# chao-ji/ldm_tf2

Hardware: AMD Instinct MI355X
Metric: images/sec (256x256, 200 DDIM steps, CFG=5) (higher is better)
Workload: dtype bf16

## Files before the change

ldm_tf2_amd/csrc/attention.hip:

```cpp
#include "common.h"
#include <atomic>
#include <stdlib.h>

namespace {

struct AttnArgs {
  const char* q; const char* k; const char* vt; char* out;
  int64_t ldq, q_bs, ldk, k_bs, ldvt, vt_bs, ldo, o_bs;
  int heads, Tq, Tk;
  float scale;
};

__device__ __forceinline__ void mma32a(f32x16& acc, const u32x4& a, const u32x4& b, bf16_t) {
  acc = __builtin_amdgcn_mfma_f32_32x32x16_bf16(__builtin_bit_cast(bf16x8, a),
                                                __builtin_bit_cast(bf16x8, b), acc, 0, 0, 0);
}
__device__ __forceinline__ void mma32a(f32x16& acc, const u32x4& a, const u32x4& b, float) {
#pragma unroll
  for (int j = 0; j < 4; ++j)
    acc = __builtin_amdgcn_mfma_f32_32x32x2f32(__uint_as_float(a[j]), __uint_as_float(b[j]), acc,
                                               0, 0, 0);
}


template <typename T>
__device__ __forceinline__ u32x4 keep_first(u32x4 v, int nvalid) {
  constexpr int EPW = 4 / (int)sizeof(T);
#pragma unroll
  for (int w = 0; w < 4; ++w) {
    const int left = nvalid - w * EPW;
    if (left <= 0) v[w] = 0u;
    else if (EPW == 2 && left == 1) v[w] &= 0xffffu;
  }
  return v;
}

template <typename T> struct AttnTraits;
template <> struct AttnTraits<bf16_t> {
  static constexpr int NPC = 2;
  __device__ static __forceinline__ int kappa(int i) {
    return (i & ~12) | ((i & 4) << 1) | ((i & 8) >> 1);
  }
  __device__ static __forceinline__ u32x4 pchunk(const f32x16& s, int pc) {
    u32x4 c;
#pragma unroll
    for (int e = 0; e < 4; ++e) c[e] = pack_bf2(s[8 * pc + 2 * e], s[8 * pc + 2 * e + 1]);
    return c;
  }
};
template <> struct AttnTraits<float> {
  static constexpr int NPC = 4;
  __device__ static __forceinline__ int kappa(int i) { return i; }
  __device__ static __forceinline__ u32x4 pchunk(const f32x16& s, int pc) {
    u32x4 c;
#pragma unroll
    for (int e = 0; e < 4; ++e) c[e] = __float_as_uint(s[4 * pc + e]);
    return c;
  }
};

template <typename T, int SP, int KT, bool MS = false, int NWV = 4, int PF = 1>
__global__ __launch_bounds__(64 * NWV, (sizeof(T) == 2 ? (SP == 32 ? 3 : SP <= 64 ? 4 : 1) : 1)) void attn_kernel(AttnArgs p) {
  constexpr int NT = 64 * NWV;
  static_assert((NWV == 4 || NWV == 8) && (PF == 1 || PF == 2), "attention workgroup shape");
  using TR = AttnTraits<T>;
  constexpr int EPC = Elem<T>::kPerChunk;
  constexpr int NPC = TR::NPC;
  constexpr int NSUB = KT / 32;
  constexpr int DCH = SP / EPC;
  constexpr int VCH = KT / EPC;
  constexpr int NKG = SP * (int)sizeof(T) / 32;
  constexpr int ND = (SP + 31) / 32;
  constexpr int KRS = SP * (int)sizeof(T) + 16;
  constexpr int VRS = KT * (int)sizeof(T) + 16;
  constexpr int CK = (KT * DCH + NT - 1) / NT;
  constexpr int CV = (SP * VCH + NT - 1) / NT;
  static_assert(SP % 16 == 0 && KT % 32 == 0 && (SP * (int)sizeof(T)) % 32 == 0, "attention tile");

  __shared__ __attribute__((aligned(16))) char smem[KT * KRS + ND * 32 * VRS];
  char* sK = smem;
  char* sV = smem + KT * KRS;

  const int tid = threadIdx.x, lane = tid & 63, wave = tid >> 6;
  const int lr = lane & 31, lh = lane >> 5;
  const int head = blockIdx.y, b = blockIdx.z;
  const int q0 = blockIdx.x * (32 * NWV) + wave * 32;

  const T* Q = (const T*)p.q + (int64_t)b * p.q_bs + (int64_t)head * SP;
  const T* Kp = (const T*)p.k + (int64_t)b * p.k_bs + (int64_t)head * SP;
  const T* Vt = (const T*)p.vt + (int64_t)b * p.vt_bs + (int64_t)head * SP * p.ldvt;

  u32x4 qf[NKG];
  {
    const int qi = min(q0 + lr, p.Tq - 1);
    const T* qr = Q + (int64_t)qi * p.ldq;
#pragma unroll
    for (int g = 0; g < NKG; ++g) qf[g] = *(const u32x4*)(qr + (2 * g + lh) * EPC);
  }

  f32x16 o[ND];
#pragma unroll
  for (int d = 0; d < ND; ++d)
#pragma unroll
    for (int r = 0; r < 16; ++r) o[d][r] = 0.f;
  constexpr int RD = 40;
  static_assert(!MS || (sizeof(T) == 2 && SP == 48), "matrix-side softmax: bf16, 40-wide heads padded to 48");
  float m_run = MS ? 0.f : -INFINITY, l_run = 0.f;
  const float c2 = p.scale * 1.4426950408889634f;

  u32x4 rkA[CK], rvA[CV];
  [[maybe_unused]] u32x4 rkB[PF == 2 ? CK : 1], rvB[PF == 2 ? CV : 1];
  auto load_tile = [&](int kt0, u32x4 (&rk)[CK], u32x4 (&rv)[CV]) {
#pragma unroll
    for (int i = 0; i < CK; ++i) {
      const int id = tid + i * NT;
      const int key = id / DCH, dc = id - key * DCH;
      u32x4 v = {0u, 0u, 0u, 0u};
      if (id < KT * DCH && kt0 + key < p.Tk)
        v = *(const u32x4*)(Kp + (int64_t)(kt0 + key) * p.ldk + dc * EPC);
      rk[i] = v;
    }
#pragma unroll
    for (int i = 0; i < CV; ++i) {
      const int id = tid + i * NT;
      const int dim = id / VCH, kc = id - dim * VCH;
      u32x4 v = {0u, 0u, 0u, 0u};
      const int left = p.Tk - (kt0 + kc * EPC);
      if (id < SP * VCH && left > 0) {
        v = *(const u32x4*)(Vt + (int64_t)dim * p.ldvt + kt0 + kc * EPC);
        if (left < EPC) v = keep_first<T>(v, left);
      }
      rv[i] = v;
    }
  };
  auto store_tile = [&](const u32x4 (&rk)[CK], const u32x4 (&rv)[CV]) {
#pragma unroll
    for (int i = 0; i < CK; ++i) {
      const int id = tid + i * NT;
      const int key = id / DCH, dc = id - key * DCH;
      if (id < KT * DCH) *(u32x4*)(sK + key * KRS + dc * 16) = rk[i];
    }
#pragma unroll
    for (int i = 0; i < CV; ++i) {
      const int id = tid + i * NT;
      const int dim = id / VCH, kc = id - dim * VCH;
      if (id < SP * VCH) *(u32x4*)(sV + dim * VRS + kc * 16) = rv[i];
    }
  };

  const int krow = TR::kappa(lr);
  const int ntiles = (p.Tk + KT - 1) / KT;
  auto tile_body = [&](int t) {
    const int kt0 = t * KT;

    f32x16 s[NSUB];
#pragma unroll
    for (int j = 0; j < NSUB; ++j) {
#pragma unroll
      for (int r = 0; r < 16; ++r) s[j][r] = 0.f;
      const char* kr = sK + (j * 32 + krow) * KRS + lh * 16;
#pragma unroll
      for (int g = 0; g < NKG; ++g) {
        const u32x4 kf = *(const u32x4*)(kr + g * 32);
        mma32a(s[j], kf, qf[g], T());
      }
    }
    if (kt0 + KT > p.Tk) {
#pragma unroll
      for (int j = 0; j < NSUB; ++j)
#pragma unroll
        for (int r = 0; r < 16; ++r) {
          const int key = kt0 + j * 32 + TR::kappa((r & 3) + 8 * (r >> 2) + 4 * lh);
          if (key >= p.Tk) s[j][r] = -INFINITY;
        }
    }
    if constexpr (MS) {
      float mt = -INFINITY;
#pragma unroll
      for (int j = 0; j < NSUB; ++j)
#pragma unroll
        for (int r = 0; r < 16; r += 2) mt = fmaxf(fmaxf(mt, s[j][r]), s[j][r + 1]);
      mt = fmaxf(mt, __shfl_xor(mt, 32, 64));
      if (t == 0 || !__all(mt <= 8.0f)) {
        const float want = m_run + (t == 0 ? mt : fmaxf(mt, 0.f));
        const float m_new = bf2f(f2bf(want));
        const float delta = m_new - m_run;
        m_run = m_new;
        if (t > 0) {
          const float alpha = __builtin_amdgcn_exp2f(-delta);
#pragma unroll
          for (int d = 0; d < ND; ++d)
#pragma unroll
            for (int r = 0; r < 16; ++r) o[d][r] *= alpha;
        }
#pragma unroll
        for (int j = 0; j < NSUB; ++j)
#pragma unroll
          for (int r = 0; r < 16; ++r) s[j][r] -= delta;
        if (lh == (RD % 16) / 8) {
          uint32_t w = qf[RD / 16][(RD % 8) / 2];
          const uint32_t nb = (uint32_t)f2bf(-m_new);
          w = (RD % 2) ? ((w & 0x0000ffffu) | (nb << 16)) : ((w & 0xffff0000u) | nb);
          qf[RD / 16][(RD % 8) / 2] = w;
        }
      }
#pragma unroll
      for (int j = 0; j < NSUB; ++j)
#pragma unroll
        for (int r = 0; r < 16; ++r) s[j][r] = __builtin_amdgcn_exp2f(s[j][r]);
    } else {
    float mt = -INFINITY;
#pragma unroll
    for (int j = 0; j < NSUB; ++j)
#pragma unroll
      for (int r = 0; r < 16; ++r) mt = fmaxf(mt, s[j][r]);
    mt = fmaxf(mt, __shfl_xor(mt, 32, 64)) * c2;
    if (!__all(mt <= m_run + 8.0f)) {
      const float m_new = fmaxf(m_run, mt);
      const float alpha = __builtin_amdgcn_exp2f(m_run - m_new);
      m_run = m_new;
      l_run *= alpha;
#pragma unroll
      for (int d = 0; d < ND; ++d)
#pragma unroll
        for (int r = 0; r < 16; ++r) o[d][r] *= alpha;
    }
    float ls = 0.f;
#pragma unroll
    for (int j = 0; j < NSUB; ++j)
#pragma unroll
      for (int r = 0; r < 16; ++r) {
        const float e = __builtin_amdgcn_exp2f(__builtin_fmaf(s[j][r], c2, -m_run));
        s[j][r] = e;
        ls += e;
      }
    l_run += ls;
    }
#pragma unroll
    for (int j = 0; j < NSUB; ++j)
#pragma unroll
      for (int pc = 0; pc < NPC; ++pc) {
        const u32x4 pf = TR::pchunk(s[j], pc);
        const int coff = (j * 2 * NPC + 2 * pc + lh) * 16;
#pragma unroll
        for (int d = 0; d < ND; ++d) {
          const u32x4 vf = *(const u32x4*)(sV + (d * 32 + lr) * VRS + coff);
          mma32a(o[d], vf, pf, T());
        }
      }
  };

  load_tile(0, rkA, rvA);
  if constexpr (PF == 2) {
    if (ntiles > 1) load_tile(KT, rkB, rvB);
    for (int t = 0; t < ntiles; t += 2) {
      __syncthreads();
      store_tile(rkA, rvA);
      __syncthreads();
      if (t + 2 < ntiles) load_tile((t + 2) * KT, rkA, rvA);
      tile_body(t);
      if (t + 1 < ntiles) {
        __syncthreads();
        store_tile(rkB, rvB);
        __syncthreads();
        if (t + 3 < ntiles) load_tile((t + 3) * KT, rkB, rvB);
        tile_body(t + 1);
      }
    }
  } else {
    for (int t = 0; t < ntiles; ++t) {
      __syncthreads();
      store_tile(rkA, rvA);
      __syncthreads();
      if (t + 1 < ntiles) load_tile((t + 1) * KT, rkA, rvA);
      tile_body(t);
    }
  }

  float l_tot;
  if constexpr (MS) {
    constexpr int RR = RD % 32;
    static_assert((RR % 8) < 4, "row RD must live in the lh = 0 half");
    l_tot = __shfl(o[RD / 32][(RR % 4) + 4 * (RR / 8)], lane & 31, 64);
  } else {
    l_tot = l_run + __shfl_xor(l_run, 32, 64);
  }
  const float inv = 1.0f / l_tot;
  const int qi = q0 + lr;
  if (qi < p.Tq) {
    T* orow = (T*)p.out + (int64_t)b * p.o_bs + (int64_t)qi * p.ldo + (int64_t)head * SP;
#pragma unroll
    for (int d = 0; d < ND; ++d)
#pragma unroll
      for (int r4 = 0; r4 < 4; ++r4) {
        const int dim = d * 32 + 8 * r4 + 4 * lh;
        if (dim >= SP) continue;
        float v[4];
#pragma unroll
        for (int e = 0; e < 4; ++e) v[e] = o[d][r4 * 4 + e] * inv;
        if constexpr (MS) {
#pragma unroll
          for (int e = 0; e < 4; ++e) v[e] = (dim + e == RD) ? 0.f : v[e];
        }
        if constexpr (sizeof(T) == 2) {
          u32x2 pk; pk[0] = pack_bf2(v[0], v[1]); pk[1] = pack_bf2(v[2], v[3]);
          *(u32x2*)(orow + dim) = pk;
        } else {
          f32x4 pk = {v[0], v[1], v[2], v[3]};
          *(f32x4*)(orow + dim) = pk;
        }
      }
  }
}



template <typename T>
__global__ __launch_bounds__(256) void attn_wide_kernel(AttnArgs p) {
  using TR = AttnTraits<T>;
  constexpr int EPC = Elem<T>::kPerChunk;
  constexpr int NPC = TR::NPC;
  constexpr int SP = 512, SPW = 128, KT = 32;
  constexpr int ES = (int)sizeof(T);
  constexpr int DCH = SP / EPC;
  constexpr int VCH = KT / EPC;
  constexpr int NKGW = SPW * ES / 32;
  constexpr int NDW = SPW / 32;
  constexpr int KRS = SP * ES + 16;
  constexpr int VRS = KT * ES + 16;
  constexpr int CK = KT * DCH / 256;
  constexpr int CV = SP * VCH / 256;
  static_assert((KT * DCH) % 256 == 0 && (SP * VCH) % 256 == 0, "staging");
  extern __shared__ __attribute__((aligned(16))) char smem_w[];
  char* sK = smem_w;
  char* sV = sK + KT * KRS;
  float* sX = (float*)(sV + SP * VRS);

  const int tid = threadIdx.x, lane = tid & 63, wave = tid >> 6;
  const int lr = lane & 31, lh = lane >> 5;
  const int head = blockIdx.y, b = blockIdx.z;
  const int q0 = blockIdx.x * 32;
  const T* Q = (const T*)p.q + (int64_t)b * p.q_bs + (int64_t)head * SP;
  const T* Kp = (const T*)p.k + (int64_t)b * p.k_bs + (int64_t)head * SP;
  const T* Vt = (const T*)p.vt + (int64_t)b * p.vt_bs + (int64_t)head * SP * p.ldvt;

  u32x4 qf[NKGW];
  {
    const int qi = min(q0 + lr, p.Tq - 1);
    const T* qr = Q + (int64_t)qi * p.ldq + wave * SPW;
#pragma unroll
    for (int g = 0; g < NKGW; ++g) qf[g] = *(const u32x4*)(qr + (2 * g + lh) * EPC);
  }
  f32x16 o[NDW];
#pragma unroll
  for (int d = 0; d < NDW; ++d)
#pragma unroll
    for (int r = 0; r < 16; ++r) o[d][r] = 0.f;
  float m_run = -INFINITY, l_run = 0.f;
  const float c2 = p.scale * 1.4426950408889634f;
  const int krow = TR::kappa(lr);
  const int ntiles = (p.Tk + KT - 1) / KT;
  for (int t = 0; t < ntiles; ++t) {
    const int kt0 = t * KT;
    __syncthreads();
#pragma unroll
    for (int i = 0; i < CK; ++i) {
      const int id = tid + i * 256;
      const int key = id / DCH, dc = id - key * DCH;
      u32x4 v = {0u, 0u, 0u, 0u};
      if (kt0 + key < p.Tk) v = *(const u32x4*)(Kp + (int64_t)(kt0 + key) * p.ldk + dc * EPC);
      *(u32x4*)(sK + key * KRS + dc * 16) = v;
    }
#pragma unroll
    for (int i = 0; i < CV; ++i) {
      const int id = tid + i * 256;
      const int dim = id / VCH, kc = id - dim * VCH;
      u32x4 v = {0u, 0u, 0u, 0u};
      const int left = p.Tk - (kt0 + kc * EPC);
      if (left > 0) {
        v = *(const u32x4*)(Vt + (int64_t)dim * p.ldvt + kt0 + kc * EPC);
        if (left < EPC) v = keep_first<T>(v, left);
      }
      *(u32x4*)(sV + dim * VRS + kc * 16) = v;
    }
    __syncthreads();
    f32x16 s;
#pragma unroll
    for (int r = 0; r < 16; ++r) s[r] = 0.f;
    {
      const char* kr = sK + krow * KRS + wave * SPW * ES + lh * 16;
#pragma unroll
      for (int g = 0; g < NKGW; ++g) {
        const u32x4 kf = *(const u32x4*)(kr + g * 32);
        mma32a(s, kf, qf[g], T());
      }
    }
    {
      float* mine = sX + (wave * 64 + lane) * 16;
#pragma unroll
      for (int r4 = 0; r4 < 4; ++r4) {
        const f32x4 v = {s[4 * r4], s[4 * r4 + 1], s[4 * r4 + 2], s[4 * r4 + 3]};
        *(f32x4*)(mine + 4 * r4) = v;
      }
      __syncthreads();
#pragma unroll
      for (int r = 0; r < 16; ++r) s[r] = 0.f;
#pragma unroll
      for (int w = 0; w < 4; ++w) {
        const float* src = sX + (w * 64 + lane) * 16;
#pragma unroll
        for (int r4 = 0; r4 < 4; ++r4) {
          const f32x4 v = *(const f32x4*)(src + 4 * r4);
#pragma unroll
          for (int e = 0; e < 4; ++e) s[4 * r4 + e] += v[e];
        }
      }
    }
    if (kt0 + KT > p.Tk) {
#pragma unroll
      for (int r = 0; r < 16; ++r) {
        const int key = kt0 + TR::kappa((r & 3) + 8 * (r >> 2) + 4 * lh);
        if (key >= p.Tk) s[r] = -INFINITY;
      }
    }
    float mt = -INFINITY;
#pragma unroll
    for (int r = 0; r < 16; ++r) mt = fmaxf(mt, s[r]);
    mt = fmaxf(mt, __shfl_xor(mt, 32, 64)) * c2;
    if (!__all(mt <= m_run + 8.0f)) {
      const float m_new = fmaxf(m_run, mt);
      const float alpha = __builtin_amdgcn_exp2f(m_run - m_new);
      m_run = m_new;
      l_run *= alpha;
#pragma unroll
      for (int d = 0; d < NDW; ++d)
#pragma unroll
        for (int r = 0; r < 16; ++r) o[d][r] *= alpha;
    }
    float ls = 0.f;
#pragma unroll
    for (int r = 0; r < 16; ++r) {
      const float e = __builtin_amdgcn_exp2f(__builtin_fmaf(s[r], c2, -m_run));
      s[r] = e;
      ls += e;
    }
    l_run += ls;
#pragma unroll
    for (int pc = 0; pc < NPC; ++pc) {
      const u32x4 pf = TR::pchunk(s, pc);
      const int coff = (2 * pc + lh) * 16;
#pragma unroll
      for (int d = 0; d < NDW; ++d) {
        const u32x4 vf = *(const u32x4*)(sV + (wave * SPW + d * 32 + lr) * VRS + coff);
        mma32a(o[d], vf, pf, T());
      }
    }
  }
  const float l_tot = l_run + __shfl_xor(l_run, 32, 64);
  const float inv = 1.0f / l_tot;
  const int qi = q0 + lr;
  if (qi < p.Tq) {
    T* orow = (T*)p.out + (int64_t)b * p.o_bs + (int64_t)qi * p.ldo + (int64_t)head * SP + wave * SPW;
#pragma unroll
    for (int d = 0; d < NDW; ++d)
#pragma unroll
      for (int r4 = 0; r4 < 4; ++r4) {
        const int dim = d * 32 + 8 * r4 + 4 * lh;
        float v[4];
#pragma unroll
        for (int e = 0; e < 4; ++e) v[e] = o[d][r4 * 4 + e] * inv;
        if constexpr (sizeof(T) == 2) {
          u32x2 pk; pk[0] = pack_bf2(v[0], v[1]); pk[1] = pack_bf2(v[2], v[3]);
          *(u32x2*)(orow + dim) = pk;
        } else {
          f32x4 pk = {v[0], v[1], v[2], v[3]};
          *(f32x4*)(orow + dim) = pk;
        }
      }
  }
}

static bool force_4_waves() {
#ifdef LDM_TOOLS_BUILD
  static const bool f = getenv("LDM_ATTN_WAVES") && atoi(getenv("LDM_ATTN_WAVES")) == 4;
  return f;
#else
  return false;
#endif
}

template <typename T>
int launch_attn_wide(const AttnArgs& a, int batch, hipStream_t s) {
  constexpr int ES = (int)sizeof(T);
  const int lds = 32 * (512 * ES + 16) + 512 * (32 * ES + 16) + 4 * 64 * 16 * 4;
  static std::atomic<uint64_t> attr_set{0};
  int devid = 0;
  if (hipGetDevice(&devid) != hipSuccess) return -1;
  const uint64_t bit = devid < 64 ? (1ull << devid) : 0;
  if (!(attr_set.load(std::memory_order_acquire) & bit) || !bit) {
    if (hipFuncSetAttribute((const void*)attn_wide_kernel<T>, hipFuncAttributeMaxDynamicSharedMemorySize, lds) != hipSuccess)
      return -1;
    attr_set.fetch_or(bit, std::memory_order_release);
  }
  dim3 grid((a.Tq + 31) / 32, a.heads, batch);
  hipLaunchKernelGGL((attn_wide_kernel<T>), grid, dim3(256), lds, s, a);
  return 0;
}

template <typename T>
int launch_attn(const AttnArgs& a, int Sp, dim3 grid, hipStream_t s) {
  constexpr bool H = sizeof(T) == 2;
#define ATTN_CASE(SPV, KTB, KTF)                                                                 \
  case SPV:                                                                                      \
    hipLaunchKernelGGL((attn_kernel<T, SPV, H ? KTB : KTF>), grid, dim3(256), 0, s, a);          \
    break;
  if constexpr (H) {
    if (Sp == 48 && a.Tq >= 256 && !force_4_waves()) {
      dim3 g8((a.Tq + 255) / 256, grid.y, grid.z);
      hipLaunchKernelGGL((attn_kernel<T, 48, 64, false, 8, 2>), g8, dim3(512), 0, s, a);
      return 0;
    }
  }
  switch (Sp) {
    ATTN_CASE(32, 128, 64)
    ATTN_CASE(48, 64, 32)
    ATTN_CASE(64, 64, 32)
    ATTN_CASE(80, 64, 32)
    ATTN_CASE(96, 64, 32)
    ATTN_CASE(160, 64, 32)
    default: return -1;
  }
#undef ATTN_CASE
  return 0;
}

}

extern "C" int ldm_attention_ms(const void* q, int64_t ldq, int64_t q_bs, const void* k, int64_t ldk,
                                int64_t k_bs, const void* vt, int64_t ldvt, int64_t vt_bs, void* out,
                                int64_t ldo, int64_t o_bs, int batch, int heads, int Tq, int Tk, int Sp,
                                int dtype, void* stream) {
  LDM_CHECK_ARG(q && k && vt && out, "ldm_attention_ms: null pointer");
  LDM_CHECK_ARG(dtype == LDM_BF16 && Sp == 48, "ldm_attention_ms: bf16 with 40-wide heads padded to 48 only");
  LDM_CHECK_ARG(batch > 0 && heads > 0 && Tq > 0 && Tk > 0 && batch < 65536 && heads < 65536, "ldm_attention_ms: bad dims");
  LDM_CHECK_ARG(ldq % 8 == 0 && ldk % 8 == 0 && ldvt % 8 == 0 && ldo % 8 == 0 && q_bs % 8 == 0 && k_bs % 8 == 0 &&
                    vt_bs % 8 == 0 && o_bs % 8 == 0 && ldvt >= Tk, "ldm_attention_ms: strides must be multiples of 8 elements, ldvt >= Tk");
  LDM_CHECK_ARG(((uintptr_t)q % 16) == 0 && ((uintptr_t)k % 16) == 0 && ((uintptr_t)vt % 16) == 0 &&
                    ((uintptr_t)out % 16) == 0, "ldm_attention_ms: pointers must be 16-byte aligned");
  AttnArgs a;
  a.q = (const char*)q; a.k = (const char*)k; a.vt = (const char*)vt; a.out = (char*)out;
  a.ldq = ldq; a.q_bs = q_bs; a.ldk = ldk; a.k_bs = k_bs; a.ldvt = ldvt; a.vt_bs = vt_bs;
  a.ldo = ldo; a.o_bs = o_bs; a.heads = heads; a.Tq = Tq; a.Tk = Tk; a.scale = 1.0f;
  if (Tq >= 256 && !force_4_waves()) {
    dim3 g8((Tq + 255) / 256, heads, batch);
    hipLaunchKernelGGL((attn_kernel<bf16_t, 48, 64, true, 8, 2>), g8, dim3(512), 0, (hipStream_t)stream, a);
  } else {
    dim3 grid((Tq + 127) / 128, heads, batch);
    hipLaunchKernelGGL((attn_kernel<bf16_t, 48, 64, true>), grid, dim3(256), 0, (hipStream_t)stream, a);
  }
  return ldm_launch_status("ldm_attention_ms");
}

extern "C" int ldm_attention(const void* q, int64_t ldq, int64_t q_bs, const void* k, int64_t ldk,
                             int64_t k_bs, const void* vt, int64_t ldvt, int64_t vt_bs, void* out,
                             int64_t ldo, int64_t o_bs, int batch, int heads, int Tq, int Tk, int Sp,
                             float scale, int dtype, void* stream) {
  LDM_CHECK_ARG(q && k && vt && out, "ldm_attention: null pointer");
  LDM_CHECK_ARG(dtype == LDM_F32 || dtype == LDM_BF16, "ldm_attention: bad dtype");
  LDM_CHECK_ARG(batch > 0 && heads > 0 && Tq > 0 && Tk > 0, "ldm_attention: bad dims");
  LDM_CHECK_ARG(batch < 65536 && heads < 65536, "ldm_attention: batch/heads too large");
  const int epc = dtype == LDM_BF16 ? 8 : 4;
  LDM_CHECK_ARG(ldq % epc == 0 && ldk % epc == 0 && ldvt % epc == 0 && ldo % epc == 0 &&
                    q_bs % epc == 0 && k_bs % epc == 0 && vt_bs % epc == 0 && o_bs % epc == 0,
                "ldm_attention: strides must be multiples of %d elements", epc);
  LDM_CHECK_ARG(ldvt >= Tk, "ldm_attention: ldvt=%lld < Tk=%d", (long long)ldvt, Tk);
  LDM_CHECK_ARG(((uintptr_t)q % 16) == 0 && ((uintptr_t)k % 16) == 0 && ((uintptr_t)vt % 16) == 0 &&
                    ((uintptr_t)out % 16) == 0, "ldm_attention: pointers must be 16-byte aligned");
  AttnArgs a;
  a.q = (const char*)q; a.k = (const char*)k; a.vt = (const char*)vt; a.out = (char*)out;
  a.ldq = ldq; a.q_bs = q_bs; a.ldk = ldk; a.k_bs = k_bs; a.ldvt = ldvt; a.vt_bs = vt_bs;
  a.ldo = ldo; a.o_bs = o_bs; a.heads = heads; a.Tq = Tq; a.Tk = Tk; a.scale = scale;
  dim3 grid((Tq + 127) / 128, heads, batch);
  hipStream_t s = (hipStream_t)stream;
  int r;
  if (Sp == 512) r = dtype == LDM_BF16 ? launch_attn_wide<bf16_t>(a, batch, s) : launch_attn_wide<float>(a, batch, s);
  else r = dtype == LDM_BF16 ? launch_attn<bf16_t>(a, Sp, grid, s) : launch_attn<float>(a, Sp, grid, s);
  LDM_CHECK_ARG(r == 0, "ldm_attention: unsupported padded head size Sp=%d (32/48/64/80/96/160, or 512 = head dim split over 4 waves)", Sp);
  return ldm_launch_status("ldm_attention");
}
```

Before: 9.131.

## Stream attention K/V tiles into a 3-stage LDS ring via buffer_load_lds

Adds a RING variant of the bf16 attention kernel that loads K and V^T tiles directly from global memory into LDS with buffer_load_lds. It uses a triple-buffered ring with swizzled layouts, so there is one barrier per tile and loads run two tiles ahead. This replaces the register-staged load/store double buffering and its two syncthreads per tile. The aim is to cut register pressure, VGPR round trips and barrier stalls. The trade-offs are a larger LDS footprint, which may lower occupancy, manual vmcnt waits that are tricky to get right, and a 2 GiB per-head size limit.

```diff
diff --git a/ldm_tf2_amd/csrc/attention.hip b/ldm_tf2_amd/csrc/attention.hip
--- a/ldm_tf2_amd/csrc/attention.hip
+++ b/ldm_tf2_amd/csrc/attention.hip
@@ -59,7 +59,7 @@
   }
 };
 
-template <typename T, int SP, int KT, bool MS = false, int NWV = 4, int PF = 1>
+template <typename T, int SP, int KT, bool MS = false, int NWV = 4, int PF = 1, bool RING = false>
 __global__ __launch_bounds__(64 * NWV, (sizeof(T) == 2 ? (SP == 32 ? 3 : SP <= 64 ? 4 : 1) : 1)) void attn_kernel(AttnArgs p) {
   constexpr int NT = 64 * NWV;
   static_assert((NWV == 4 || NWV == 8) && (PF == 1 || PF == 2), "attention workgroup shape");
@@ -77,7 +77,11 @@
   constexpr int CV = (SP * VCH + NT - 1) / NT;
   static_assert(SP % 16 == 0 && KT % 32 == 0 && (SP * (int)sizeof(T)) % 32 == 0, "attention tile");
 
-  __shared__ __attribute__((aligned(16))) char smem[KT * KRS + ND * 32 * VRS];
+  static_assert(!RING || (sizeof(T) == 2 && (KT == 64 || KT == 128)), "attention ring: bf16, 64- or 128-key tiles");
+  constexpr int KIMG = SP * KT * (int)sizeof(T);
+  constexpr int NPK = KIMG / 1024;
+  constexpr int NRS = 3;
+  __shared__ __attribute__((aligned(16))) char smem[RING ? NRS * 2 * KIMG : KT * KRS + ND * 32 * VRS];
   char* sK = smem;
   char* sV = smem + KT * KRS;
 
@@ -108,8 +112,8 @@
   float m_run = MS ? 0.f : -INFINITY, l_run = 0.f;
   const float c2 = p.scale * 1.4426950408889634f;
 
-  u32x4 rkA[CK], rvA[CV];
-  [[maybe_unused]] u32x4 rkB[PF == 2 ? CK : 1], rvB[PF == 2 ? CV : 1];
+  [[maybe_unused]] u32x4 rkA[RING ? 1 : CK], rvA[RING ? 1 : CV];
+  [[maybe_unused]] u32x4 rkB[PF == 2 && !RING ? CK : 1], rvB[PF == 2 && !RING ? CV : 1];
   auto load_tile = [&](int kt0, u32x4 (&rk)[CK], u32x4 (&rv)[CV]) {
 #pragma unroll
     for (int i = 0; i < CK; ++i) {
@@ -150,7 +154,21 @@
 
   const int krow = TR::kappa(lr);
   const int ntiles = (p.Tk + KT - 1) / KT;
-  auto tile_body = [&](int t) {
+  const int koff = RING ? krow * 32 + ((lh ^ ((krow >> 3) & 1)) << 4) : krow * KRS + lh * 16;
+  auto kfrag = [&](const char* base, int j, int g) -> u32x4 {
+    if constexpr (RING) return *(const u32x4*)(base + g * (KT * 32) + j * 1024 + koff);
+    else return *(const u32x4*)(base + j * 32 * KRS + g * 32 + koff);
+  };
+  auto vfrag = [&](const char* base, int d, int cc) -> u32x4 {
+    if constexpr (RING) {
+      const int row = d * 32 + ((SP % 32 != 0 && d == ND - 1) ? (lr & 15) : lr);
+      const int x = KT == 64 ? (lr >> 1) & 7 : lr & 15;
+      return *(const u32x4*)(base + row * (KT * 2) + ((cc ^ x) << 4));
+    } else {
+      return *(const u32x4*)(base + (d * 32 + lr) * VRS + cc * 16);
+    }
+  };
+  auto tile_body = [&](int t, const char* tK, const char* tV) {
     const int kt0 = t * KT;
 
     f32x16 s[NSUB];
@@ -158,12 +176,8 @@
     for (int j = 0; j < NSUB; ++j) {
 #pragma unroll
       for (int r = 0; r < 16; ++r) s[j][r] = 0.f;
-      const char* kr = sK + (j * 32 + krow) * KRS + lh * 16;
-#pragma unroll
-      for (int g = 0; g < NKG; ++g) {
-        const u32x4 kf = *(const u32x4*)(kr + g * 32);
-        mma32a(s[j], kf, qf[g], T());
-      }
+#pragma unroll
+      for (int g = 0; g < NKG; ++g) mma32a(s[j], kfrag(tK, j, g), qf[g], T());
     }
     if (kt0 + KT > p.Tk) {
 #pragma unroll
@@ -241,15 +255,90 @@
 #pragma unroll
       for (int pc = 0; pc < NPC; ++pc) {
         const u32x4 pf = TR::pchunk(s[j], pc);
-        const int coff = (j * 2 * NPC + 2 * pc + lh) * 16;
-#pragma unroll
-        for (int d = 0; d < ND; ++d) {
-          const u32x4 vf = *(const u32x4*)(sV + (d * 32 + lr) * VRS + coff);
-          mma32a(o[d], vf, pf, T());
-        }
+        const int cc = j * 2 * NPC + 2 * pc + lh;
+#pragma unroll
+        for (int d = 0; d < ND; ++d) mma32a(o[d], vfrag(tV, d, cc), pf, T());
       }
   };
 
+  if constexpr (RING) {
+    typedef __attribute__((address_space(3))) void* lds_ptr;
+    constexpr uint32_t kOOB = 0x80000000u;
+    constexpr int NP = 2 * NPK;
+    constexpr int CMAX = (NP + NWV - 1) / NWV;
+    const int wv = __builtin_amdgcn_readfirstlane(wave);
+    const __amdgpu_buffer_rsrc_t rsK = __builtin_amdgcn_make_buffer_rsrc(
+        const_cast<T*>(Kp), 0, (uint32_t)((int64_t)p.Tk * p.ldk * (int64_t)sizeof(T)), 0x00020000);
+    const __amdgpu_buffer_rsrc_t rsV = __builtin_amdgcn_make_buffer_rsrc(
+        const_cast<T*>(Vt), 0, (uint32_t)((int64_t)SP * p.ldvt * (int64_t)sizeof(T)), 0x00020000);
+    uint32_t off0[CMAX];
+    int rel[CMAX];
+#pragma unroll
+    for (int i = 0; i < CMAX; ++i) {
+      const int n = i * NWV + wv;
+      if (n < NPK) {
+        const int g = n / (KT / 32), key = (n % (KT / 32)) * 32 + (lane >> 1);
+        const int h = (lane & 1) ^ ((key >> 3) & 1);
+        off0[i] = (uint32_t)(key * p.ldk + g * 16 + h * 8) * (uint32_t)sizeof(T);
+        rel[i] = key;
+      } else {
+        constexpr int VCH = KT / 8;
+        const int r = (n - NPK) * (1024 / (KT * 2)) + lane / VCH;
+        const int cc = (lane % VCH) ^ (VCH == 8 ? (r >> 1) & 7 : r & 15);
+        off0[i] = (uint32_t)(r * p.ldvt + cc * 8) * (uint32_t)sizeof(T);
+        rel[i] = cc * 8;
+      }
+    }
+    auto issue = [&](int t, char* stg) {
+      const int kt0 = t * KT;
+#pragma unroll
+      for (int i = 0; i < CMAX; ++i) {
+        const int n = i * NWV + wv;
+        if (n < NP) {
+          const bool isk = n < NPK;
+          const uint32_t step = isk ? (uint32_t)(kt0 * p.ldk * (int64_t)sizeof(T)) : (uint32_t)(kt0 * sizeof(T));
+          const uint32_t off = kt0 + rel[i] < p.Tk ? off0[i] + step : kOOB;
+          __builtin_amdgcn_raw_ptr_buffer_load_lds(isk ? rsK : rsV, (lds_ptr)(stg + n * 1024), 16, off, 0, 0, 0);
+        }
+      }
+    };
+    auto wait_tile = [&](int t, char* stg) {
+      if (t + 1 < ntiles) {
+        if (wv < NP % NWV || NP % NWV == 0) asm volatile("s_waitcnt vmcnt(%0)" ::"n"(CMAX) : "memory");
+        else asm volatile("s_waitcnt vmcnt(%0)" ::"n"(CMAX - 1) : "memory");
+      } else {
+        asm volatile("s_waitcnt vmcnt(0)" ::: "memory");
+      }
+      const int kt0 = t * KT;
+      if (kt0 + KT > p.Tk) {
+#pragma unroll
+        for (int i = 0; i < CMAX; ++i) {
+          const int n = i * NWV + wv;
+          const int left = p.Tk - (kt0 + rel[i]);
+          if (n >= NPK && n < NP && left > 0 && left < EPC) {
+            u32x4* c = (u32x4*)(stg + n * 1024 + lane * 16);
+            *c = keep_first<T>(*c, left);
+          }
+        }
+        asm volatile("s_waitcnt lgkmcnt(0)" ::: "memory");
+      }
+    };
+    issue(0, smem);
+    if (ntiles > 1) issue(1, smem + 2 * KIMG);
+#pragma unroll
+    for (int g = 0; g < NKG; ++g) asm volatile("" : "+v"(qf[g]));
+    int st = 0;
+    for (int t = 0; t < ntiles; ++t) {
+      char* cur = smem + st * (2 * KIMG);
+      wait_tile(t, cur);
+      __builtin_amdgcn_s_barrier();
+      asm volatile("" ::: "memory");
+      const int s2 = st == 0 ? 2 : st - 1;
+      if (t + 2 < ntiles) issue(t + 2, smem + s2 * (2 * KIMG));
+      tile_body(t, cur, cur + KIMG);
+      st = st == 2 ? 0 : st + 1;
+    }
+  } else {
   load_tile(0, rkA, rvA);
   if constexpr (PF == 2) {
     if (ntiles > 1) load_tile(KT, rkB, rvB);
@@ -258,13 +347,13 @@
       store_tile(rkA, rvA);
       __syncthreads();
       if (t + 2 < ntiles) load_tile((t + 2) * KT, rkA, rvA);
-      tile_body(t);
+      tile_body(t, sK, sV);
       if (t + 1 < ntiles) {
         __syncthreads();
         store_tile(rkB, rvB);
         __syncthreads();
         if (t + 3 < ntiles) load_tile((t + 3) * KT, rkB, rvB);
-        tile_body(t + 1);
+        tile_body(t + 1, sK, sV);
       }
     }
   } else {
@@ -273,8 +362,9 @@
       store_tile(rkA, rvA);
       __syncthreads();
       if (t + 1 < ntiles) load_tile((t + 1) * KT, rkA, rvA);
-      tile_body(t);
-    }
+      tile_body(t, sK, sV);
+    }
+  }
   }
 
   float l_tot;
@@ -507,17 +597,30 @@
   return 0;
 }
 
-template <typename T>
-int launch_attn(const AttnArgs& a, int Sp, dim3 grid, hipStream_t s) {
+static bool ring_off() {
+#ifdef LDM_TOOLS_BUILD
+  static const bool f = getenv("LDM_ATTN_RING") && atoi(getenv("LDM_ATTN_RING")) == 0;
+  return f;
+#else
+  return false;
+#endif
+}
+
+static bool ring_fits(const AttnArgs& a, int Sp, int es) {
+  return (int64_t)a.Tk * a.ldk * es < 0x80000000ll && (int64_t)Sp * a.ldvt * es < 0x80000000ll;
+}
+
+template <typename T, bool RING>
+int launch_attn_form(const AttnArgs& a, int Sp, dim3 grid, hipStream_t s) {
   constexpr bool H = sizeof(T) == 2;
 #define ATTN_CASE(SPV, KTB, KTF)                                                                 \
   case SPV:                                                                                      \
-    hipLaunchKernelGGL((attn_kernel<T, SPV, H ? KTB : KTF>), grid, dim3(256), 0, s, a);          \
+    hipLaunchKernelGGL((attn_kernel<T, SPV, H ? KTB : KTF, false, 4, 1, RING>), grid, dim3(256), 0, s, a); \
     break;
   if constexpr (H) {
     if (Sp == 48 && a.Tq >= 256 && !force_4_waves()) {
       dim3 g8((a.Tq + 255) / 256, grid.y, grid.z);
-      hipLaunchKernelGGL((attn_kernel<T, 48, 64, false, 8, 2>), g8, dim3(512), 0, s, a);
+      hipLaunchKernelGGL((attn_kernel<T, 48, 64, false, 8, 2, RING>), g8, dim3(512), 0, s, a);
       return 0;
     }
   }
@@ -532,6 +635,19 @@
   }
 #undef ATTN_CASE
   return 0;
+}
+
+template <typename T>
+int launch_attn(const AttnArgs& a, int Sp, dim3 grid, hipStream_t s) {
+  if constexpr (sizeof(T) == 2) {
+#ifdef LDM_TOOLS_BUILD
+    if (ring_off()) return launch_attn_form<T, false>(a, Sp, grid, s);
+#endif
+    if (!ring_fits(a, Sp, 2)) return -2;
+    return launch_attn_form<T, true>(a, Sp, grid, s);
+  } else {
+    return launch_attn_form<T, false>(a, Sp, grid, s);
+  }
 }
 
 }
@@ -551,13 +667,19 @@
   a.q = (const char*)q; a.k = (const char*)k; a.vt = (const char*)vt; a.out = (char*)out;
   a.ldq = ldq; a.q_bs = q_bs; a.ldk = ldk; a.k_bs = k_bs; a.ldvt = ldvt; a.vt_bs = vt_bs;
   a.ldo = ldo; a.o_bs = o_bs; a.heads = heads; a.Tq = Tq; a.Tk = Tk; a.scale = 1.0f;
-  if (Tq >= 256 && !force_4_waves()) {
-    dim3 g8((Tq + 255) / 256, heads, batch);
-    hipLaunchKernelGGL((attn_kernel<bf16_t, 48, 64, true, 8, 2>), g8, dim3(512), 0, (hipStream_t)stream, a);
-  } else {
-    dim3 grid((Tq + 127) / 128, heads, batch);
-    hipLaunchKernelGGL((attn_kernel<bf16_t, 48, 64, true>), grid, dim3(256), 0, (hipStream_t)stream, a);
-  }
+  LDM_CHECK_ARG(ring_fits(a, Sp, 2), "ldm_attention_ms: K or V^T of one head spans 2 GiB or more");
+  const hipStream_t s = (hipStream_t)stream;
+  const bool w8 = Tq >= 256 && !force_4_waves();
+  const dim3 grid((Tq + (w8 ? 255 : 127)) / (w8 ? 256 : 128), heads, batch);
+#ifdef LDM_TOOLS_BUILD
+  if (ring_off()) {
+    if (w8) hipLaunchKernelGGL((attn_kernel<bf16_t, 48, 64, true, 8, 2>), grid, dim3(512), 0, s, a);
+    else hipLaunchKernelGGL((attn_kernel<bf16_t, 48, 64, true>), grid, dim3(256), 0, s, a);
+    return ldm_launch_status("ldm_attention_ms");
+  }
+#endif
+  if (w8) hipLaunchKernelGGL((attn_kernel<bf16_t, 48, 64, true, 8, 1, true>), grid, dim3(512), 0, s, a);
+  else hipLaunchKernelGGL((attn_kernel<bf16_t, 48, 64, true, 4, 1, true>), grid, dim3(256), 0, s, a);
   return ldm_launch_status("ldm_attention_ms");
 }
 
@@ -585,6 +707,7 @@
   int r;
   if (Sp == 512) r = dtype == LDM_BF16 ? launch_attn_wide<bf16_t>(a, batch, s) : launch_attn_wide<float>(a, batch, s);
   else r = dtype == LDM_BF16 ? launch_attn<bf16_t>(a, Sp, grid, s) : launch_attn<float>(a, Sp, grid, s);
+  LDM_CHECK_ARG(r != -2, "ldm_attention: K or V^T of one head spans 2 GiB or more");
   LDM_CHECK_ARG(r == 0, "ldm_attention: unsupported padded head size Sp=%d (32/48/64/80/96/160, or 512 = head dim split over 4 waves)", Sp);
   return ldm_launch_status("ldm_attention");
 }
```

After: 9.156 (median of 6 runs). Within noise of the previous version (+0.3%).
